# yifanlu0227/HEAL

Measured on AMD Instinct MI355X. Metric: scenes/sec (5-agent OPV2V-H, PointPillars+PyramidFusion), higher is better.
Workload: dtype f32

## Files before the change

### heal_amd/_capi.py

```python
import ctypes
import os
import re

HERE = os.path.dirname(os.path.abspath(__file__))
LIB_PATH = os.environ.get("HEAL_AMD_LIB") or os.path.join(HERE, "lib", "libheal_amd.so")
HEADER = os.path.join(os.path.dirname(HERE), "include", "heal_amd.h")
HEADER_EXPERIMENTAL = os.path.join(os.path.dirname(HERE), "include", "heal_amd_experimental.h")

_lib = None

c_void_p, c_int, c_float, c_size_t = ctypes.c_void_p, ctypes.c_int, ctypes.c_float, ctypes.c_size_t

_SIGNATURES = {
    "heal_abi_version": (c_int, []),
    "heal_last_error": (ctypes.c_char_p, []),
    "heal_fill_bytes": (c_int, [c_void_p, c_int, c_size_t, c_void_p]),
    "heal_next_launch_events": (c_int, [c_void_p, c_void_p]),
    "heal_voxelize_workspace": (c_size_t, [c_int, c_int, c_int, ctypes.c_longlong]),
    "heal_voxelize": (c_int, [c_void_p, c_int, c_void_p, c_void_p, c_int, c_int, c_int,
                              c_void_p, c_void_p, c_void_p, c_void_p, c_void_p, c_void_p, c_void_p, c_size_t, c_int, c_void_p]),
    "heal_voxelize_batch_workspace": (c_size_t, [c_int, c_int, c_int, c_int, ctypes.c_longlong]),
    "heal_voxelize_batch": (c_int, [c_void_p, c_void_p, c_int, c_void_p, c_void_p, c_int, c_int, c_void_p, c_void_p,
                                    c_void_p, c_void_p, c_void_p, c_size_t, c_int, c_void_p]),
    "heal_mask_points": (c_int, [c_void_p, c_int, c_void_p, c_int, c_void_p, c_void_p]),
# ... 44 lines not shown
                                  c_float, c_float, c_float, c_float, c_void_p, c_void_p]),
    "heal_pfn_moments": (c_int, [c_void_p, c_void_p, c_void_p, c_int, c_int, c_float, c_float, c_float, c_float, c_float, c_float,
                                 c_void_p, c_void_p]),
    "heal_pfn_backward": (c_int, [c_void_p, c_void_p, c_void_p, c_int, c_int, c_void_p, c_void_p, c_void_p, c_void_p, c_void_p,
                                  c_float, c_float, c_float, c_float, c_float, c_float, c_void_p, c_void_p, c_void_p]),
    "heal_mean_vfe": (c_int, [c_void_p, c_void_p, c_int, c_int, c_int, c_void_p, c_void_p, c_void_p]),
    "heal_sp_sort_workspace": (c_size_t, [c_int]),
    "heal_sp_sort_sites": (c_int, [c_void_p, c_int, c_void_p, c_int, c_void_p, c_void_p, c_void_p, c_size_t, c_void_p,
                                   c_void_p]),
    "heal_sp_wgrad_chunks": (c_int, [c_int]),
    "heal_sp_wgrad": (c_int, [c_void_p, c_void_p, c_void_p, c_int, c_int, c_int, c_int, c_void_p, c_void_p, c_void_p]),
    "heal_sp_gather_rows": (c_int, [c_void_p, c_void_p, c_int, c_int, c_void_p, c_void_p, c_void_p]),
    "heal_sp_table_capacity": (c_size_t, [c_int]),
    "heal_sp_hash_build": (c_int, [c_void_p, c_int, c_void_p, c_int, c_void_p, c_void_p, c_size_t, c_void_p, c_void_p]),
    "heal_sp_neighbors": (c_int, [c_void_p, c_int, c_void_p, c_void_p, c_void_p, c_void_p, c_void_p, c_int,
                                  c_void_p, c_void_p, c_size_t, c_void_p, c_void_p, c_void_p]),
    "heal_sp_out_sites_workspace": (c_size_t, [c_int, c_int]),
    "heal_sp_out_sites": (c_int, [c_void_p, c_int, c_void_p, c_void_p, c_void_p, c_void_p, c_void_p, c_int,
                                  c_void_p, c_int, c_void_p, c_void_p, c_size_t, c_void_p, c_void_p]),
    "heal_conv_gemm": (c_int, [c_void_p, c_void_p, c_void_p, c_void_p] + [c_int] * 8 + [c_void_p, c_void_p]),
    "heal_ln_stats": (c_int, [c_void_p, c_int, c_int, c_float, c_void_p, c_void_p]),
    "heal_linear": (c_int, [c_void_p, c_int, c_int, ctypes.c_longlong, c_void_p, c_void_p, c_void_p, c_int, c_void_p, c_int,
                            c_int, c_void_p, c_int, c_void_p, c_int, c_int, c_int, c_int, c_int, c_int, c_int,
                            ctypes.c_longlong, c_int, c_void_p]),
    "heal_split_attn_workspace": (c_size_t, [c_int, c_int, c_int]),
    "heal_split_attn_weights": (c_int, [c_void_p, ctypes.c_longlong, c_int, c_int, c_int] + [c_void_p] * 5 + [c_float] +
                                [c_void_p] * 5),
    "heal_split_attn_colsum": (c_int, [c_void_p, ctypes.c_longlong, c_int, c_int, c_int, c_void_p, c_void_p]),
    "heal_split_attn_weights_from_colsum": (c_int, [c_void_p, c_int, c_int, c_int, c_int] + [c_void_p] * 5 + [c_float] +
                                            [c_void_p] * 4),
    "heal_sp_rank_bytes": (c_size_t, [c_void_p, c_int]),
    "heal_sp_out_sites_rank": (c_int, [c_void_p, c_int, c_void_p, c_void_p, c_void_p, c_void_p, c_void_p, c_int,
                                       c_void_p, c_int, c_void_p, c_void_p, c_size_t, c_void_p, c_void_p, c_void_p]),
    "heal_sp_neighbors_rank": (c_int, [c_void_p, c_int, c_void_p, c_void_p, c_void_p, c_void_p, c_void_p, c_int,
                                       c_void_p, c_size_t, c_int, c_void_p, c_void_p, c_void_p, c_void_p]),
    "heal_sp_neighbors_root": (c_int, [c_void_p, c_int, c_void_p, c_void_p, c_void_p, c_void_p, c_void_p, c_int,
                                       c_void_p, c_size_t, c_int, c_void_p, c_void_p, c_void_p, c_void_p]),
    "heal_sp_root_rank_bytes": (c_size_t, [c_void_p, c_int]),
    "heal_sp_pair_tiles_words": (c_size_t, [c_int, c_int]),
    "heal_sp_neighbor_tiles": (c_int, [c_void_p, c_int, c_void_p, c_void_p, c_void_p, c_void_p, c_void_p, c_int,
                                       c_void_p, c_size_t, c_int, c_int, c_void_p, c_int, c_void_p, c_void_p, c_void_p]),
    "heal_sp_tiles_to_neighbors": (c_int, [c_void_p, c_int, c_int, c_void_p, c_void_p, c_void_p]),
    "heal_sp_conv_tiles_supported": (c_int, [c_int, c_int]),
    "heal_sp_conv_tiles": (c_int, [c_void_p, c_void_p, c_int, c_int, c_int, c_int, c_void_p, c_void_p, c_void_p, c_int,
                                   c_void_p, c_void_p, c_void_p]),
    "heal_sp_root_rank": (c_int, [c_void_p, c_int, c_void_p, c_int, c_void_p, c_void_p, c_void_p, c_int, c_void_p, c_void_p,
                                  c_size_t, c_void_p, c_void_p]),
    "heal_gconv_conv3_supported": (c_int, [c_int] * 5),
    "heal_gconv_conv3": (c_int, [c_void_p] * 6 + [c_int] * 7 + [c_void_p, c_void_p]),
    "heal_sp_transpose_neighbors": (c_int, [c_void_p, c_int, c_int, c_int, c_void_p, c_void_p, c_void_p]),
    "heal_sp_weight_fragments": (c_int, [c_void_p, c_int, c_int, c_int, c_void_p, c_void_p]),
    "heal_sp_conv": (c_int, [c_void_p, c_void_p, c_int, c_int, c_int, c_int, c_void_p, c_void_p, c_void_p, c_void_p, c_int,
                             c_void_p, c_void_p, c_void_p]),
    "heal_sp_to_bev_workspace": (c_size_t, [c_int, c_int, c_int, c_int]),
    "heal_sp_to_bev": (c_int, [c_void_p, c_void_p, c_int, c_int, c_void_p, c_int, c_void_p, c_void_p, c_size_t,
                               c_void_p, c_void_p]),
    "heal_agent_attention": (c_int, [c_void_p, c_void_p, c_void_p, c_void_p, c_int, c_int, c_int, c_int, c_float,
                                     c_int, c_void_p, c_int, c_void_p]),
    "heal_agent_attention_backward": (c_int, [c_void_p] * 5 + [c_int, c_int, c_int, c_int, c_float, c_int] + [c_void_p] * 3 +
                                      [c_int, c_void_p]),
    "heal_grouped_conv3x3": (c_int, [c_void_p, c_void_p, c_void_p, c_int, c_int, c_int, c_int, c_int, c_int, c_int,
                                     c_void_p, c_void_p]),
    "heal_bias_act": (c_int, [c_void_p, c_void_p, c_void_p, c_int, c_int, c_int, c_int, c_void_p]),
    "heal_resnext_bottleneck": (c_int, [c_void_p] * 7 + [c_int, c_int, c_int, c_int, c_void_p, c_void_p]),
    "heal_upsample2x_bilinear": (c_int, [c_void_p, c_int, c_int, c_int, c_int, c_void_p, c_void_p]),
    "heal_depthwise_conv": (c_int, [c_void_p, c_void_p, c_void_p] + [c_int] * 11 + [c_void_p, c_void_p, c_void_p]),
    "heal_camera_matrices": (c_int, [c_void_p] * 5 + [c_int, c_void_p, c_void_p]),
    "heal_channel_dot": (c_int, [c_void_p] * 3 + [c_int] * 3 + [c_void_p, c_void_p]),
    "heal_layernorm_nchw": (c_int, [c_void_p] * 3 + [c_int] * 3 + [c_float, c_void_p, c_void_p]),
    "heal_se_gate": (c_int, [c_void_p] * 5 + [c_int] * 3 + [c_float, c_int, c_void_p, c_void_p]),
    "heal_conv1x1": (c_int, [c_void_p] * 5 + [c_int] * 8 + [c_void_p, c_void_p]),
    "heal_stem7x7": (c_int, [c_void_p, ctypes.c_longlong, c_int, c_int, c_int, c_int, c_void_p, c_void_p, c_int, c_void_p, c_void_p]),
    "heal_conv1x1_split_supported": (c_int, [c_int] * 4),
    "heal_conv1x1_split": (c_int, [c_void_p] * 4 + [c_int] * 7 + [c_void_p, c_void_p]),
    "heal_conv1x1_tiled_supported": (c_int, [c_int] * 5),
    "heal_conv1x1_tiled": (c_int, [c_void_p] * 4 + [c_int] * 9 + [c_void_p, c_void_p]),
    "heal_conv1x1_splitk_workspace": (c_size_t, [c_int] * 5),
    "heal_conv1x1_splitk": (c_int, [c_void_p] * 5 + [c_int] * 7 + [c_void_p, c_void_p, c_size_t, c_void_p]),
    "heal_conv1x1_d2s": (c_int, [c_void_p] * 3 + [c_int] * 9 + [c_void_p, c_void_p]),
    "heal_conv3x3": (c_int, [c_void_p] * 4 + [c_int] * 7 + [c_void_p, c_void_p]),
    "heal_conv3x3_same": (c_int, [c_void_p] * 3 + [c_int] * 11 + [c_void_p, c_void_p]),
    "heal_grouped16_conv3x3": (c_int, [c_void_p] * 3 + [c_int] * 5 + [c_void_p, c_void_p]),
    "heal_grouped_small_conv3x3": (c_int, [c_void_p] * 3 + [c_int] * 7 + [c_void_p, c_void_p]),
    "heal_conv3x3_winograd4": (c_int, [c_void_p] * 4 + [c_int] * 6 + [c_void_p, c_void_p]),
    "heal_conv3x3_winograd": (c_int, [c_void_p] * 4 + [c_int] * 7 + [c_void_p, c_void_p]),
    "heal_conv3x3_winograd_kc": (c_int, [c_void_p] * 4 + [c_int] * 8 + [c_void_p, c_void_p]),
    "heal_conv3x3_winograd_splitk_workspace": (c_size_t, [c_int] * 5),
    "heal_conv3x3_winograd_splitk": (c_int, [c_void_p] * 4 + [c_int] * 8 + [c_void_p, c_void_p, c_size_t, c_void_p]),
    "heal_nms_quads_workspace": (c_size_t, [c_int]),
    "heal_nms_quads": (c_int, [c_void_p, c_int, c_float, c_void_p, c_size_t, c_void_p, c_void_p, c_void_p]),
    "heal_window_attention": (c_int, [c_void_p, c_void_p, c_int, c_int, c_int, c_int, c_int, c_int, c_float, c_void_p,
                                      c_void_p]),
    "heal_window_attention_backward_workspace": (c_size_t, [c_int, c_int, c_int, c_int]),
    "heal_window_attention_backward": (c_int, [c_void_p] * 4 + [c_int] * 6 + [c_float, c_void_p, c_void_p, c_void_p, c_size_t,
                                                c_void_p]),
    "heal_agent_window_attention": (c_int, [c_void_p, c_void_p] + [c_int] * 8 + [c_float, c_void_p, c_void_p]),
    "heal_agent_mean": (c_int, [c_void_p, c_int, ctypes.c_longlong, c_void_p, c_void_p]),
    "heal_v2v_message_workspace": (c_size_t, [c_int] * 5),
    "heal_v2v_message": (c_int, [c_void_p, c_void_p, c_void_p, ctypes.c_longlong, c_void_p, c_void_p] + [c_int] * 9
                         + [c_void_p, c_void_p, c_size_t, c_void_p]),
    "heal_gru_zero_state": (c_int, [c_void_p, ctypes.c_longlong, c_void_p, ctypes.c_longlong] + [c_int] * 4 + [c_void_p, c_void_p]),
    "heal_label_assign_workspace": (c_size_t, [c_int]),
    "heal_label_assign": (c_int, [c_void_p, c_int, c_void_p, c_int, c_float, c_float, c_void_p, c_void_p, c_void_p,
                                  c_size_t, c_void_p]),
    "heal_boxes_bev_matrix": (c_int, [c_void_p, c_int, c_void_p, c_int, c_int, c_void_p, c_void_p]),
    "heal_nms_bev_workspace": (c_size_t, [c_int]),
    "heal_nms_bev": (c_int, [c_void_p, c_int, c_float, c_int, c_void_p, c_size_t, c_void_p, c_void_p, c_void_p]),
    "heal_kd_kl_loss_workspace": (c_size_t, [c_int] * 4),
    "heal_kd_kl_loss": (c_int, [c_void_p, c_void_p] + [c_int] * 4 + [c_void_p, c_void_p, c_void_p, c_size_t, c_void_p]),
}


class HealAmdError(RuntimeError):
    pass


def declared_symbols(experimental=False):
    text = open(HEADER_EXPERIMENTAL if experimental else HEADER).read()
    text = re.sub(r"/\*.*?\*/", "", text, flags=re.S)
    return sorted(set(re.findall(r"\b(heal_[a-z0-9_]+)\s*\(", text)))


def abi_version_of_header():
    m = re.search(r"#define\s+HEAL_AMD_ABI_VERSION\s+(\d+)", open(HEADER).read())
    if not m:
        raise HealAmdError(f"{HEADER} does not define HEAL_AMD_ABI_VERSION")
    return int(m.group(1))


def lib():
    global _lib
    if _lib is None:
        if not os.path.exists(LIB_PATH):
            raise HealAmdError(
                f"{LIB_PATH} is missing: the HIP extension has not been built "
                "(run `python -m heal_amd.build`); heal_amd has no CPU fallback")
        import torch
        L = ctypes.CDLL(LIB_PATH)
        for name, (res, args) in _SIGNATURES.items():
            if not hasattr(L, name):
                continue
            f = getattr(L, name)
            f.restype = res
            f.argtypes = args
        want = abi_version_of_header()
        got = int(L.heal_abi_version()) if hasattr(L, "heal_abi_version") else -1
        if got != want:
            raise HealAmdError(f"{LIB_PATH} has C-ABI version {got}, include/heal_amd.h declares {want}: rebuild it "
                               "(python -m heal_amd.build --force)")
        _lib = L
    return _lib


_TRACE = int(os.environ.get("HEAL_TRACE_CALLS", "0") or 0)


def _trace_call(name, args):
    import sys
    import torch
    cap = torch.cuda.is_current_stream_capturing()
    extra = ""
    if _TRACE >= 2:
        extra = " " + " ".join(hex(a.value or 0) if isinstance(a, ctypes.c_void_p) else str(a) for a in args
                               if isinstance(a, (int, float, ctypes.c_void_p)))
    print(f"[heal pid {os.getpid()}] {'capture ' if cap else ''}{name}{extra}", file=sys.stderr, flush=True)

# ... 103 lines not shown
```

### heal_amd/opencood/models/sub_modules/bev_blocks.py

```python
import numpy as np
import torch
import torch.nn as nn
import torch.nn.functional as F

from heal_amd.derived import derived


def fold_bn(conv, bn, transposed=False):
    def build():
        scale = bn.weight / torch.sqrt(bn.running_var + bn.eps)
        shift = bn.bias - bn.running_mean * scale
        if transposed:
            w = conv.weight * scale.view(1, -1, 1, 1)
        else:
            w = conv.weight * scale.view(-1, 1, 1, 1)
        b = shift if conv.bias is None else shift + conv.bias * scale
        return w.contiguous(), b.contiguous()
    return derived("fold_bn", (conv.weight, conv.bias, bn.weight, bn.bias, bn.running_mean, bn.running_var), build, (transposed,))


import os
_CONV1X1 = os.environ.get("HEAL_CONV1X1", "1") == "1"
_CONV3X3 = os.environ.get("HEAL_CONV3X3", "1") == "1"

# ... 59 lines not shown
    if module.training and torch.is_grad_enabled():
        raise NotImplementedError(
            f"{type(module).__name__}: no gradient path (the sparse-convolution encoder is inference-only in this build). "
            "Call model.eval() and run under torch.no_grad(), or freeze this module (eval mode, input without gradient).")


class ConvBN(nn.Module):

    @staticmethod
    def run(x, conv, bn, relu, residual=None, out=None):
        if out is not None and not grad_path(x, bn, conv):
            w, b = fold_bn(conv, bn)
            y = conv_bias_act(x, w, b, conv.stride, conv.padding, conv.dilation, conv.groups, relu, residual, out=out)
            if y.data_ptr() != out.data_ptr():
                out.copy_(y)
            return out
        if out is not None:
            return out.copy_(ConvBN.run(x, conv, bn, relu, residual))
        if grad_path(x, bn, conv):
            y = bn(conv(x))
            if residual is not None:
                y = y + residual
            return F.relu(y) if relu else y
        w, b = fold_bn(conv, bn)
        return conv_bias_act(x, w, b, conv.stride, conv.padding, conv.dilation, conv.groups, relu, residual)


def conv3x3(in_planes, out_planes, stride=1, groups=1, dilation=1):
    return nn.Conv2d(in_planes, out_planes, kernel_size=3, stride=stride, padding=dilation, groups=groups,
                     bias=False, dilation=dilation)


def conv1x1(in_planes, out_planes, stride=1):
    return nn.Conv2d(in_planes, out_planes, kernel_size=1, stride=stride, bias=False)


class BasicBlock(nn.Module):
    expansion = 1

    def __init__(self, inplanes, planes, stride=1, downsample=None, groups=1, base_width=64, dilation=1,
                 norm_layer=None):
        super().__init__()
        norm_layer = norm_layer or nn.BatchNorm2d
        if groups != 1 or base_width != 64:
            raise ValueError("BasicBlock only supports groups=1 and base_width=64")
        self.conv1 = conv3x3(inplanes, planes, stride)
        self.bn1 = norm_layer(planes)
        self.relu = nn.ReLU(inplace=True)
        self.conv2 = conv3x3(planes, planes)
        self.bn2 = norm_layer(planes)
        self.downsample = downsample
        self.stride = stride

    def takes_pooled(self):
        d = self.downsample
        return (d is not None and isinstance(d[0], nn.Conv2d) and d[0].kernel_size == (1, 1) and d[0].stride == (2, 2)
                and d[0].padding == (0, 0) and d[0].out_channels == 64 and d[0].bias is None
                and self.conv1.stride == (2, 2) and self.conv1.out_channels == 64 and self.conv1.in_channels % 32 == 0
                and isinstance(self.bn1, nn.BatchNorm2d) and isinstance(d[1], nn.BatchNorm2d))

    def _stem_params(self, x):
        from heal_amd import ops
        w1, b1 = fold_bn(self.conv1, self.bn1)
        wd, bd = fold_bn(self.downsample[0], self.downsample[1])
        frag = getattr(x, "fragments", ops.stem_fragments)
        return derived("stem_block", (w1, b1, wd, bd), lambda: frag(w1, wd) + (b1, bd), (getattr(x, "weight_layout", "tiles"),))

    def forward(self, x):
        from heal_amd import ops
        if isinstance(x, (ops.PooledBEV, ops.PillarBEV)):
            if (not grad_path(None, self) and self.takes_pooled() and x.channels == self.conv1.in_channels
                    and x.stem_supported(self.conv1.out_channels, self.downsample[0].out_channels)):
                wm, wd, b1, bd = self._stem_params(x)
                out, identity = x.stem_block(wm, b1, wd, bd)
                return ConvBN.run(out, self.conv2, self.bn2, relu=True, residual=identity)
            x = x.dense()
        identity = x
        if self.downsample is not None:
            identity = ConvBN.run(x, self.downsample[0], self.downsample[1], relu=False)
        out = ConvBN.run(x, self.conv1, self.bn1, relu=True)
        return ConvBN.run(out, self.conv2, self.bn2, relu=True, residual=identity)


class Bottleneck(nn.Module):
    expansion = 4

    def __init__(self, inplanes, planes, stride=1, downsample=None, groups=1, base_width=64, dilation=1,
                 norm_layer=None, expansion=None):
        super().__init__()
        norm_layer = norm_layer or nn.BatchNorm2d
        exp = self.expansion if expansion is None else expansion
        width = int(planes * (base_width / 64.0)) * groups
        self.conv1 = conv1x1(inplanes, width)
        self.bn1 = norm_layer(width)
        self.conv2 = conv3x3(width, width, stride, groups, dilation)
        self.bn2 = norm_layer(width)
        self.conv3 = conv1x1(width, planes * exp)
        self.bn3 = norm_layer(planes * exp)
        self.relu = nn.ReLU(inplace=True)
        self.downsample = downsample
        self.stride = stride

    def _fused_params(self):
        from heal_amd import ops
        w1, b1 = fold_bn(self.conv1, self.bn1)
        w2, b2 = fold_bn(self.conv2, self.bn2)
        w3, b3 = fold_bn(self.conv3, self.bn3)
        return derived("resnext_bottleneck", (w1, b1, w2, b2, w3, b3), lambda: (
            ops.mfma_a_fragments(w1.reshape(w1.shape[0], w1.shape[1])), b1, w2, b2,
            ops.mfma_a_fragments(w3.reshape(w3.shape[0], w3.shape[1])), b3))

    def _fusable(self, x):
        import os
        if os.environ.get("HEAL_FUSED_BOTTLENECK", "0") != "1":
            return False
        from heal_amd import ops
        if not ops.experimental_build():
            return False
        c = self.conv1.in_channels
        return (x.is_cuda and self.downsample is None and self.stride == 1 and self.conv2.groups == 32
                and self.conv3.out_channels == c and self.conv1.out_channels == 2 * c and c in (64, 128, 256)
                and self.conv2.dilation == (1, 1))

    def out_shape(self, x):
        s = self.stride
        return (int(x.shape[0]), self.conv3.out_channels, (int(x.shape[2]) - 1) // s + 1, (int(x.shape[3]) - 1) // s + 1)

    def forward(self, x, out=None):
        if not grad_path(x, self) and self._fusable(x):
            from heal_amd import ops
            y = ops.resnext_bottleneck(x.contiguous(), *self._fused_params())
            return y if out is None else out.copy_(y)
        identity = x
        if self.downsample is not None:
            identity = ConvBN.run(x, self.downsample[0], self.downsample[1], relu=False)
        y = ConvBN.run(x, self.conv1, self.bn1, relu=True)
        y = ConvBN.run(y, self.conv2, self.bn2, relu=True)
        return ConvBN.run(y, self.conv3, self.bn3, relu=True, residual=identity, out=out)


class ResNetModified(nn.Module):

    def __init__(self, block, layers, layer_strides, num_filters, groups=1, width_per_group=64, inplanes=64,
                 expansion=None):
        super().__init__()
        self.inplanes = inplanes
        self.groups = groups
        self.base_width = width_per_group
        self.layernum = len(num_filters)
        self._exp = block.expansion if expansion is None else expansion
        for i in range(self.layernum):
            setattr(self, f"layer{i}", self._make_layer(block, num_filters[i], layers[i], layer_strides[i]))
        for m in self.modules():
            if isinstance(m, nn.Conv2d):
                nn.init.kaiming_normal_(m.weight, mode="fan_out", nonlinearity="relu")

    def _make_layer(self, block, planes, blocks, stride):
        exp = self._exp
        kw = {"expansion": exp} if block is Bottleneck else {}
        downsample = None
        if stride != 1 or self.inplanes != planes * exp:
            downsample = nn.Sequential(conv1x1(self.inplanes, planes * exp, stride), nn.BatchNorm2d(planes * exp))
        layers = [block(self.inplanes, planes, stride, downsample, self.groups, self.base_width, 1, None, **kw)]
        self.inplanes = planes * exp
        for _ in range(1, blocks):
            layers.append(block(self.inplanes, planes, groups=self.groups, base_width=self.base_width, **kw))
        return nn.Sequential(*layers)

    @staticmethod
    def stage_chunk(layer, x):
        mb = float(os.environ.get("HEAL_STAGE_CHUNK_MB", "0"))
        if mb <= 0 or not x.is_cuda or torch.is_grad_enabled() or not all(isinstance(b, Bottleneck) for b in layer):
            return 0
        n = int(x.shape[0])
        blk = layer[-1]
        co, s0 = blk.conv3.out_channels, layer[0].stride
        ho, wo = (int(x.shape[2]) - 1) // s0 + 1, (int(x.shape[3]) - 1) // s0 + 1
        per_agent = 4.0 * ho * wo * (2 * co + 2 * blk.conv1.out_channels) / 2 ** 20
        chunk = max(1, int(mb // per_agent))
        return chunk if chunk < n else 0

    def run_stage(self, layer, x):
        chunk = self.stage_chunk(layer, x)
        if not chunk:
            return layer(x)
        n = int(x.shape[0])
        shape = list(x.shape)
        for blk in layer:
            shape = list(blk.out_shape(torch.empty(shape, device="meta")))
        y = torch.empty(shape, dtype=x.dtype, device=x.device)
        for a in range(0, n, chunk):
            xa = x[a:a + chunk]
            for j, blk in enumerate(layer):
                xa = blk(xa, out=y[a:a + chunk]) if j == len(layer) - 1 else blk(xa)
        return y

    def forward(self, x):
        feats = []
        for i in range(self.layernum):
            x = self.run_stage(getattr(self, f"layer{i}"), x)
            feats.append(x)
        return feats


class _Deblock(nn.Sequential):

    def __init__(self, conv, bn):
        super().__init__(conv, bn, nn.ReLU())

    def out_shape(self, x):
        conv = self[0]
        if isinstance(conv, nn.ConvTranspose2d):
            return conv.out_channels, int(x.shape[2]) * conv.stride[0], int(x.shape[3]) * conv.stride[1]
        s0, s1 = conv.stride
        return conv.out_channels, (int(x.shape[2]) - conv.kernel_size[0]) // s0 + 1, (int(x.shape[3]) - conv.kernel_size[1]) // s1 + 1

    def forward(self, x, into=None):
        y = self._forward(x, into)
        if into is not None and y.data_ptr() != into[0][:, into[1]:].data_ptr():
            dst = into[0][:, into[1]:into[1] + y.shape[1]]
# ... 253 lines not shown
```

### heal_amd/ops.py

```python
import ctypes
import os

import numpy as np
import torch

from . import _capi, derived
from .derived import derived as _derived

_WS = {}

TIMING = None
SP_TRACE = None
LAST_CALLS = None


def _remember(name, fn):
    if LAST_CALLS is not None:
        LAST_CALLS[name] = fn


def graph_period_ms(fn, reps=20, iters=10):
    global TIMING, LAST_CALLS
    saved = (TIMING, LAST_CALLS)
    TIMING, LAST_CALLS = None, None
# ... 1687 lines not shown


def split_attn_weights(branches, groups, rows_per_group, w_out, b_out, fc1, ln_g, ln_b, eps, fc2):
    branches = _need(branches, torch.float32, "branches")
    C = int(branches.shape[-1])
    dev = branches.device
    ws = _workspace("split_attn", _capi.query("heal_split_attn_workspace", groups, rows_per_group, C), dev)
    scale = torch.empty((groups, 3, C), dtype=torch.float32, device=dev)
    bias = torch.empty((groups, C), dtype=torch.float32, device=dev)
    _capi.call("heal_split_attn_weights", _ptr(branches), int(branches.stride(0)), groups, rows_per_group, C, _ptr(w_out),
               _ptr(b_out), _ptr(fc1), _ptr(ln_g), _ptr(ln_b), float(eps), _ptr(fc2), _ptr(ws), _ptr(scale), _ptr(bias),
               _stream())
    return scale, bias


def split_attn_colsum(branches, groups, rows_per_group):
    branches = _need(branches, torch.float32, "branches")
    C = int(branches.shape[-1])
    out = torch.empty((groups, 3, (rows_per_group + 511) // 512, C), dtype=torch.float32, device=branches.device)
    _capi.call("heal_split_attn_colsum", _ptr(branches), int(branches.stride(0)), groups, rows_per_group, C, _ptr(out), _stream())
    return out


def split_attn_weights_from_colsum(colsum, rows_per_part, w_out, b_out, fc1, ln_g, ln_b, eps, fc2):
    colsum = _need(colsum, torch.float32, "colsum")
    n_parts, groups, _three, chunks, C = (int(v) for v in colsum.shape)
    if chunks != (rows_per_part + 511) // 512:
        raise ValueError(f"split_attn_weights_from_colsum: {chunks} chunks do not match {rows_per_part} rows per part")
    dev = colsum.device
    scale = torch.empty((groups, 3, C), dtype=torch.float32, device=dev)
    bias = torch.empty((groups, C), dtype=torch.float32, device=dev)
    _capi.call("heal_split_attn_weights_from_colsum", _ptr(colsum), n_parts, groups, int(rows_per_part), C, _ptr(w_out),
               _ptr(b_out), _ptr(fc1), _ptr(ln_g), _ptr(ln_b), float(eps), _ptr(fc2), _ptr(scale), _ptr(bias), _stream())
    return scale, bias


def grouped16_fragments(weight, cg):
    def build():
        C = int(weight.shape[0])
        w = weight.detach().reshape(C // 16, 16, cg, 9)
        if cg == 16:
            full = w
        else:
            full = torch.zeros((C // 16, 16, 16, 9), dtype=w.dtype, device=w.device)
            full[:, :8, :8] = w[:, :8]
            full[:, 8:, 8:] = w[:, 8:]
        return full.reshape(C // 16, 16, 4, 4, 9).permute(0, 4, 2, 3, 1).contiguous()
    return _derived("grouped16_fragments", (weight,), build)


def grouped_small_fragments(weight, cg):
    C = int(weight.shape[0])
    return _derived("grouped_small_fragments", (weight,),
                    lambda: weight.detach().reshape(C // 16, 16, cg, 9).permute(0, 3, 2, 1).contiguous())


def grouped_conv3x3(x, weight, bias, groups, stride=1, relu=True):
    import os
    x = _need(x, torch.float32, "x")
    weight = _need(weight, torch.float32, "weight")
    n, C, H, W = (int(v) for v in x.shape)
    bias = _need_bias(bias, C, "grouped_conv3x3")
    Ho, Wo = (H + 2 - 3) // stride + 1, (W + 2 - 3) // stride + 1
    y = torch.empty((n, C, Ho, Wo), dtype=torch.float32, device=x.device)
    cg = C // groups
    mode = os.environ.get("HEAL_GCONV_MFMA", "1")
    if C % 16 == 0 and W % 4 == 0 and Wo % 4 == 0 and mode in ("1", "s") and cg in (4, 8, 16):
        frag = grouped_small_fragments(weight, cg)
        with _Timed(f"grouped_conv3x3_c{C}" + ("_s2" if stride == 2 else ""), 2.0 * 9 * n * C * cg * Ho * Wo,
                    4.0 * n * C * (H * W + Ho * Wo), kernel_events=True):
            _capi.call("heal_grouped_small_conv3x3", _ptr(x), _ptr(frag), _ptr(bias), n, C, cg, H, W, int(stride),
                       int(bool(relu)), _ptr(y), _stream())
        return y
    if stride == 1 and C % 16 == 0 and W % 4 == 0 and ((cg == 16 and mode != "0") or (cg == 8 and mode == "8")):
        frag = grouped16_fragments(weight, cg)
        with _Timed(f"grouped_conv3x3_c{C}", 2.0 * 9 * n * C * cg * Ho * Wo, 4.0 * n * C * (H * W + Ho * Wo)):
            _capi.call("heal_grouped16_conv3x3", _ptr(x), _ptr(frag), _ptr(bias), n, C, H, W, int(bool(relu)), _ptr(y),
                       _stream())
        return y
    with _Timed(f"grouped_conv3x3_c{C}" + ("_s2" if stride == 2 else ""), 2.0 * 9 * n * C * (C // groups) * Ho * Wo,
                4.0 * n * C * (H * W + Ho * Wo)):
        _capi.call("heal_grouped_conv3x3", _ptr(x), _ptr(weight), _ptr(bias), n, C, int(groups), H, W, int(stride),
                   int(bool(relu)), _ptr(y), _stream())
    return y


def gconv_conv3_supported(width, cg, cout, H, W):
    return bool(_capi.query("heal_gconv_conv3_supported", int(width), int(cg), int(cout), int(H), int(W)))


def gconv_conv3(x, w2, b2, groups, w3, b3, residual=None, relu=True):
    x = _need(x, torch.float32, "x")
    n, width, H, W = (int(v) for v in x.shape)
    cg = width // groups
    cout = int(w3.shape[0])
    frag2 = grouped_small_fragments(_need(w2, torch.float32, "w2"), cg)
    frag3 = _derived("gconv_conv3_fragments", (w3,), lambda: mfma_a_fragments(w3.detach().reshape(cout, width)))
    y = torch.empty((n, cout, H, W), dtype=torch.float32, device=x.device)
    flops = 2.0 * n * H * W * (9 * width * cg + width * cout)
    nbytes = 4.0 * n * H * W * (width + cout * (2 if residual is not None else 1))
    with _Timed(f"gconv_conv3_{width}_{cout}", flops, nbytes, kernel_events=True):
        _capi.call("heal_gconv_conv3", _ptr(x), _ptr(frag2), _ptr(_need(b2, torch.float32, "b2")), _ptr(frag3),
                   _ptr(_need(b3, torch.float32, "b3")), _optr(residual), n, width, cg, cout, H, W, int(bool(relu)), _ptr(y), _stream())
    return y


def bias_act_(x, bias=None, residual=None, relu=True):
    x = _need(x, torch.float32, "x")
    n, C = int(x.shape[0]), int(x.shape[1])
    HW = int(x.shape[2] * x.shape[3])
    if residual is not None:
        residual = _need(residual, torch.float32, "residual")
    _capi.call("heal_bias_act", _ptr(x), _ptr(bias), _ptr(residual), n, C, HW, int(bool(relu)), _stream())
    return x


def mfma_a_fragments(wm):
    M, K = wm.shape
    return wm.reshape(M // 16, 16, K // 4, 4).permute(0, 2, 3, 1).reshape(M // 16, K // 4, 64).contiguous()


def conv1x1_fragments(w):
    def build():
        cout, cin = int(w.shape[0]), int(w.shape[1])
        mpad, kpad = (cout + 63) // 64 * 64, (cin + 31) // 32 * 32
        wm = w.detach().reshape(cout, cin)
        if (mpad, kpad) != (cout, cin):
            wm = torch.nn.functional.pad(wm, (0, kpad - cin, 0, mpad - cout))
        fr = mfma_a_fragments(wm)
        return fr.reshape(mpad // 16, kpad // 16, 4, 64).permute(0, 1, 3, 2).contiguous()
    return _derived("conv1x1_fragments", (w,), build)


def conv1x1_supported(cin, cout, hw, stride=1, out_w=None):
    if stride == 1:
        return hw % 4 == 0 and hw >= 64
    return stride == 2 and out_w is not None and out_w % 4 == 0 and hw >= 64


def conv1x1_ksplit(n, cin, cout, hw):
    chunks = (cin + 31) // 32
    blocks = -(-cout // 64) * -(-hw // 64) * n
    env = os.environ.get("HEAL_C1_KSPLIT")
    want = int(env) if env is not None else (min(chunks // 2, max(2, 256 // blocks)) if blocks < 128 and chunks >= 8 else 1)
    if want < 2 or chunks < 2 or hw % 4:
        return 1
    want = min(want, chunks, 65535 // n)
    return -(-chunks // -(-chunks // want))


def stem7x7_fragments(w):
    cout, cin = int(w.shape[0]), int(w.shape[1])
    if cout != 64 or tuple(w.shape[2:]) != (7, 7) or not 1 <= cin <= 4:
        raise _capi.HealAmdError(f"stem7x7: weight must be [64, 1..4, 7, 7], got {tuple(w.shape)}")

    def build():
        K = cin * 49
        ks = (K + 3) // 4
        wk = torch.nn.functional.pad(w.detach().to(torch.float32).reshape(64, K), (0, 4 * ks - K))
        return wk.reshape(4, 16, ks, 4).permute(0, 2, 3, 1).contiguous()
    return _derived("stem7x7_fragments", (w,), build)


def stem7x7(x, w, bias, pool=True):
    x = _need(x, torch.float32, "x")
    n, cx, H, W = (int(v) for v in x.shape)
# ... 425 lines not shown
```

### include/heal_amd.h

```cpp
#ifndef HEAL_AMD_H
#define HEAL_AMD_H

#include <stddef.h>
#include <stdint.h>

#ifdef __cplusplus
extern "C" {
#endif

#define HEAL_AMD_ABI_VERSION 12

int heal_abi_version(void);
const char* heal_last_error(void);

int heal_fill_bytes(void* dst, int byte, size_t bytes, void* stream);
int heal_next_launch_events(void* start_event, void* stop_event);

size_t heal_voxelize_workspace(int n_points, int max_points, int max_voxels, long long agents_x_cells);
int heal_voxelize(const float* points, int n_points,
                  const float* range_host, const float* voxel_size_host,
                  int max_points, int max_voxels, int batch_idx,
                  float* voxels, int32_t* coords, int32_t* num_points, int32_t* n_voxels,
                  const int32_t* row_offset, int32_t* row_offset_next,
                  void* ws, size_t ws_bytes, int tables_clean, void* stream);
// ... 162 lines not shown
int heal_sp_conv_tiles(const float* feat_in, const uint32_t* tiles, int n_out, int slot_sites, int c_in, int c_out,
                       const float* weight_frag, const float* bn_scale, const float* bn_shift, int relu, float* feat_out,
                       const int32_t* n_out_dev, void* stream);
int heal_sp_transpose_neighbors(const int32_t* nbr, int n_out, int kernel_volume, int n_in, int32_t* nbr_t,
                                const int32_t* n_out_dev, void* stream);
int heal_sp_wgrad_chunks(int n_out);
int heal_sp_wgrad(const float* feat_in, const float* grad_out, const int32_t* nbr, int n_out, int kernel_volume, int c_in,
                  int c_out, const int32_t* n_out_dev, float* partials, void* stream);
int heal_sp_weight_fragments(const float* weight, int kernel_volume, int c_in, int c_out, float* out, void* stream);
int heal_sp_conv(const float* feat_in, const int32_t* nbr, int n_out, int kernel_volume, int c_in, int c_out,
                 const float* weight, const float* weight_frag, const float* bn_scale, const float* bn_shift,
                 int relu, float* feat_out, const int32_t* n_out_dev, void* stream);
size_t heal_sp_to_bev_workspace(int batch, int D, int H, int W);
int heal_sp_to_bev(const float* features, const int32_t* indices, int n, int channels,
                   const int32_t* shape_host, int batch, float* out, void* ws, size_t ws_bytes,
                   const int32_t* n_dev, void* stream);

int heal_bev_pool_backward(const float* grad_cells, const float* depth_logit, const float* feat, const float* frustum,
                           const float* cam_mats, int n_agents, int n_cams, int D, int fH, int fW, int channels,
                           const float* dx_host, const float* bx_host, const int32_t* nx_host, float* grad_logit,
                           float* grad_feat, void* stream);

int heal_agent_attention(const float* q, const float* k, const float* v, const int32_t* key_mask, int n_pix,
                         int n_agents, int channels, int heads, float scale, int out_rows, float* out,
                         int agent_major ,
                         void* stream);
int heal_agent_attention_backward(const float* q, const float* k, const float* v, const int32_t* key_mask,
                                  const float* grad_out, int n_pix, int n_agents, int channels, int heads, float scale,
                                  int out_rows, float* grad_q, float* grad_k, float* grad_v, int agent_major, void* stream);

int heal_grouped_conv3x3(const float* x, const float* weight, const float* bias, int n, int channels, int groups,
                         int H, int W, int stride, int relu, float* y, void* stream);
int heal_bias_act(float* x, const float* bias, const float* residual, int n, int channels, int HW, int relu,
                  void* stream);

int heal_upsample2x_bilinear(const float* x, int n, int channels, int H, int W, float* y, void* stream);

int heal_depthwise_conv(const float* x, const float* weight, const float* bias, int n, int channels, int H, int W,
                        int ksize, int stride, int pad_t, int pad_l, int Ho, int Wo, int act, float* y,
                        float* channel_sums, void* stream);

int heal_layernorm_nchw(const float* x, const float* gamma, const float* beta, int n, int channels, int HW, float eps,
                        float* y, void* stream);

int heal_channel_dot(const float* x, const float* weight, const float* bias, int n, int channels, int HW, float* y,
                     void* stream);

int heal_se_gate(const float* mean, const float* w_reduce, const float* b_reduce, const float* w_expand_t,
                 const float* b_expand, int n, int channels, int squeezed, float scale, int tiles, float* gate,
                 void* stream);

int heal_conv1x1(const float* x, const float* weight_frag, const float* bias, const float* residual,
                 const float* in_scale, int n, int cin, int cout, int H, int W, int stride, int act,
                 int out_pixel_major, float* y, void* stream);

int heal_conv3x3_same(const float* x, const float* weight_frag, const float* bias, int n, int cin, int cout, int H, int W,
                      int stride, int pad_t, int pad_l, int Ho, int Wo, int act, float* y, void* stream);

int heal_stem7x7(const float* x, long long image_stride, int n, int cin, int H, int W, const float* weight_frag,
                 const float* bias, int pool, float* y, void* stream);
int heal_conv1x1_split_supported(int cin, int cout, int H, int W);
int heal_conv1x1_split(const float* x, const void* weight_frag, const float* bias, const float* residual, int n, int cin, int cout,
                       int H, int W, int act, int n_products, float* y, void* stream);
size_t heal_conv1x1_splitk_workspace(int n, int cout, int H, int W, int ksplit);
int heal_conv1x1_splitk(const float* x, const float* weight_frag, const float* bias, const float* residual,
                        const float* in_scale, int n, int cin, int cout, int H, int W, int act, int ksplit, float* y, void* ws,
                        size_t ws_bytes, void* stream);

int heal_conv1x1_d2s(const float* x, const float* weight_frag, const float* bias, int n, int cin, int cout, int H, int W,
                     int act, int k, int dst_channels, int dst_channel_offset, float* y, void* stream);

int heal_conv3x3(const float* x, const float* weight_frag, const float* bias, const float* residual, int n, int cin,
                 int cout, int H, int W, int stride, int relu, float* y, void* stream);

int heal_conv_gemm(const float* x, const float* weight_tap_major, const float* bias, const float* residual, int n, int cin,
                   int cout, int H, int W, int ksize, int stride, int relu, float* y, void* stream);

int heal_grouped16_conv3x3(const float* x, const float* weight_frag, const float* bias, int n, int channels, int H, int W,
                           int relu, float* y, void* stream);

int heal_grouped_small_conv3x3(const float* x, const float* weight_q, const float* bias, int n, int channels,
                               int group_channels, int H, int W, int stride, int relu, float* y, void* stream);

int heal_conv3x3_winograd(const float* x, const float* u_frag, const float* bias, const float* residual, int n, int cin,
                          int cout, int H, int W, int relu, int waves, float* y, void* stream);
int heal_conv3x3_winograd_kc(const float* x, const float* u_frag, const float* bias, const float* residual, int n, int cin,
                             int cout, int H, int W, int relu, int waves, int kc, float* y, void* stream);
size_t heal_conv3x3_winograd_splitk_workspace(int n, int cout, int H, int W, int ksplit);
int heal_conv3x3_winograd_splitk(const float* x, const float* u_frag, const float* bias, const float* residual, int n, int cin,
                                 int cout, int H, int W, int relu, int waves, int ksplit, float* y, void* ws, size_t ws_bytes,
                                 void* stream);

int heal_boxes_bev_matrix(const float* boxes_a, int n, const float* boxes_b, int m, int mode, float* out,
                          void* stream);
size_t heal_nms_bev_workspace(int n);
int heal_nms_bev(const float* boxes_sorted, int n, float thresh, int rotated, void* workspace,
                 size_t workspace_bytes, long long* keep, int* num_keep, void* stream);

size_t heal_nms_quads_workspace(int n);
int heal_nms_quads(const float* quads_sorted, int n, float thresh, void* workspace, size_t workspace_bytes,
                   long long* keep, int* num_keep, void* stream);

int heal_window_attention(const float* qkv, const float* pos_bias, int n_agents, int H, int W, int heads,
                          int dim_head, int window, float scale, float* out, void* stream);
size_t heal_window_attention_backward_workspace(int n_agents, int H, int W, int heads);
int heal_window_attention_backward(const float* qkv, const float* pos_bias, const float* out, const float* grad_out, int n_agents,
                                   int H, int W, int heads, int dim_head, int window, float scale, float* grad_qkv,
                                   float* grad_bias, void* ws, size_t ws_bytes, void* stream);

int heal_agent_window_attention(const float* qkv, const float* bias, int n_agents, int n_valid, int H, int W, int heads,
                                int dim_head, int window, int mode, float scale, float* out, void* stream);
int heal_agent_mean(const float* x, int n_agents, long long n_elems, float* out, void* stream);

size_t heal_v2v_message_workspace(int n_ego, int cout, int H, int W, int nsplit);
int heal_v2v_message(const float* xs, const float* mask, const float* e, long long e_stride, const float* w_frag,
                     const float* residual, int n_ego, int n_agents, int cin, int cout, int H, int W, int mode, int nsplit,
                     int tile_h, float* out, void* ws, size_t ws_bytes, void* stream);
int heal_gru_zero_state(const float* gates, long long gates_stride, const float* add, long long add_stride, int n, int channels,
                        int H, int W, float* h, void* stream);

int heal_ln_stats(const float* x, int n_tokens, int channels, float eps, float* stats, void* stream);
int heal_linear(const float* x, int lda, int x_part_cols, long long x_part_stride, const float* ln_stats,
                const float* weight, const float* bias,
                int bias_per_group, const float* colscale, int colscale_part, int group_rows, const float* residual,
                int ldr, float* out, int ldo, int n_tokens, int n_out, int n_in, int map_inner, int map_outer,
                int part_cols, long long part_stride, int act, void* stream);
size_t heal_split_attn_workspace(int groups, int rows_per_group, int channels);
int heal_split_attn_weights(const float* branches, long long part_stride, int groups, int rows_per_group, int channels,
                            const float* w_out, const float* b_out, const float* fc1, const float* ln_gamma,
                            const float* ln_beta, float eps, const float* fc2, float* colsum_ws, float* scale,
                            float* bias, void* stream);
int heal_split_attn_colsum(const float* branches, long long part_stride, int groups, int rows_per_group, int channels,
                           float* colsum, void* stream);
int heal_split_attn_weights_from_colsum(const float* colsum, int n_parts, int groups, int rows_per_part, int channels,
                                        const float* w_out, const float* b_out, const float* fc1, const float* ln_gamma,
                                        const float* ln_beta, float eps, const float* fc2, float* scale, float* bias,
                                        void* stream);

size_t heal_label_assign_workspace(int n_gt);
int heal_label_assign(const float* anchor_boxes, int n_anchors, const float* gt_boxes, int n_gt,
                      float pos_threshold, float neg_threshold, int32_t* assigned, uint8_t* neg, void* ws,
                      size_t ws_bytes, void* stream);

size_t heal_kd_kl_loss_workspace(int n, int channels, int H, int W);
int heal_kd_kl_loss(const float* student, const float* teacher, int n, int channels, int H, int W, float* loss, float* grad,
                    void* ws, size_t ws_bytes, void* stream);

#ifdef __cplusplus
}
#endif
#endif
```

Measured before the change: 161.2.

## Fuse bottleneck 1x1 conv with grouped 3x3 conv in one HIP kernel

Adds a kernel that computes the bottleneck's conv1 (1x1, BN-folded, ReLU) for a haloed tile into LDS with MFMA, then immediately runs the 32-group 3x3 conv2 from LDS, for specific ResNeXt block shapes. This removes the global-memory write and re-read of the intermediate activation and one kernel launch. In exchange the halo pixels of conv1 are recomputed across neighbouring tiles. The path is gated on a fixed set of shapes and environment flags.

```diff
diff --git a/heal_amd/_capi.py b/heal_amd/_capi.py
--- a/heal_amd/_capi.py
+++ b/heal_amd/_capi.py
@@ -150,6 +150,7 @@
     "heal_conv3x3_same": (c_int, [c_void_p] * 3 + [c_int] * 11 + [c_void_p, c_void_p]),
     "heal_grouped16_conv3x3": (c_int, [c_void_p] * 3 + [c_int] * 5 + [c_void_p, c_void_p]),
     "heal_grouped_small_conv3x3": (c_int, [c_void_p] * 3 + [c_int] * 7 + [c_void_p, c_void_p]),
+    "heal_conv1_gconv3x3": (c_int, [c_void_p] * 5 + [c_int] * 7 + [c_void_p, c_void_p]),
     "heal_conv3x3_winograd4": (c_int, [c_void_p] * 4 + [c_int] * 6 + [c_void_p, c_void_p]),
     "heal_conv3x3_winograd": (c_int, [c_void_p] * 4 + [c_int] * 7 + [c_void_p, c_void_p]),
     "heal_conv3x3_winograd_kc": (c_int, [c_void_p] * 4 + [c_int] * 8 + [c_void_p, c_void_p]),
diff --git a/heal_amd/csrc/conv1_gconv.hip b/heal_amd/csrc/conv1_gconv.hip
--- /dev/null
+++ b/heal_amd/csrc/conv1_gconv.hip
@@ -0,0 +1,235 @@
+#include <stdlib.h>
+#include "common.h"
+#include "../../include/heal_amd.h"
+
+namespace heal {
+
+using f32x4 = __attribute__((ext_vector_type(4))) float;
+
+template <int CG, int TH, int STRIDE, int PF>
+__global__ __launch_bounds__(256) __attribute__((amdgpu_waves_per_eu(PF == 1 && TH == 8 && STRIDE == 1 ? 4 : 3, PF == 1 && TH == 8 && STRIDE == 1 ? 5 : 4))) void k_conv1_gconv(
+    const float* __restrict__ x, const float* __restrict__ w1frag, const float* __restrict__ b1, const float* __restrict__ wq,
+    const float* __restrict__ b2, int Cin, int width, int H, int W, int Ho, int Wo, int tiles_x, float* __restrict__ y) {
+    static_assert(CG == 4 || CG == 8 || CG == 16, "4, 8 or 16 channels per group");
+    static_assert(TH == 8 || TH == 16, "tile height");
+    static_assert(STRIDE == 1 || STRIDE == 2, "stride");
+    static_assert(PF == 1 || PF == 2, "chunks in flight per block");
+    constexpr int TW = STRIDE == 1 ? 32 : 16, NSEG = TW / 16, RW = TH / 4;
+    constexpr int PR = STRIDE * TH + 3 - STRIDE, PC = STRIDE * TW + 3 - STRIDE;
+    constexpr int NSIDE = 3 - STRIDE;
+    constexpr int NSTEP = 9 * CG;
+    constexpr int KH = CG == 16 ? 2 : 1;
+    constexpr int CGH = CG / KH;
+    constexpr int NB = CG / 4, NBH = CGH / 4;
+    static_assert(STRIDE * TW == 32, "a patch row is 32 interior pixels + halo");
+    constexpr int KC = 8;
+    constexpr int RS = 36;
+    constexpr int LD = (PR * RS - 16 + 31) / 32 * 32 + 16;
+    constexpr int NPIX = PR * PC, NT = (NPIX + 15) / 16, NTW = (NT + 3) / 4;
+    constexpr int SP4 = NPIX * 4, SX4 = 2 * KC * LD / 4, SA4 = SP4 > SX4 ? SP4 : SX4, SW4 = NSTEP * 16 / 4;
+    static_assert((SA4 + SW4) * 16 <= 80 * 1024, "two blocks per CU");
+    __shared__ float4 smem[SA4 + SW4];
+    float4* const sP = smem;
+    float* const sX = reinterpret_cast<float*>(smem);
+    float4* const sW = smem + SA4;
+
+    const Block3 bk = xcd_block();
+    const int sg = bk.x, n = bk.z;
+    const int ty = bk.y / tiles_x, tx = bk.y - ty * tiles_x;
+    const int oy0 = ty * TH, ox0 = tx * TW;
+    const int gy0 = oy0 * STRIDE - 1, gx0 = ox0 * STRIDE;
+    const int t = threadIdx.x, wave = t >> 6, l = t & 63;
+    const int lk = l >> 4, ln = l & 15;
+    const size_t HW = (size_t)H * W, HWo = (size_t)Ho * Wo;
+    const float* __restrict__ xin = x + (size_t)n * Cin * HW;
+
+    constexpr int IT_W = (SW4 + 255) / 256;
+#pragma unroll
+    for (int it = 0; it < IT_W; ++it) {
+        const int i = min(t + 256 * it, SW4 - 1);
+        sW[i] = reinterpret_cast<const float4*>(wq + (size_t)sg * NSTEP * 16)[i];
+    }
+
+    constexpr int N_IN = PR * KC * 8, IT_IN = (N_IN + 255) / 256;
+    constexpr int N_HA = PR * KC * NSIDE, IT_HA = (N_HA + 255) / 256;
+    int g_in[IT_IN], s_in[IT_IN], g_ha[IT_HA], s_ha[IT_HA];
+#pragma unroll
+    for (int it = 0; it < IT_IN; ++it) {
+        const int u = min(t + 256 * it, N_IN - 1);
+        const int quad = u & 7, ch = (u >> 3) & 7, row = u >> 6;
+        const int gy = gy0 + row, gx = gx0 + quad * 4;
+        const bool ok = gy >= 0 && gy < H && gx < W;
+        g_in[it] = ch * (int)HW + (ok ? gy * W + gx : 0);
+        s_in[it] = ch * LD + row * RS + quad * 4;
+    }
+#pragma unroll
+    for (int it = 0; it < IT_HA; ++it) {
+        const int u = min(t + 256 * it, N_HA - 1);
+        const int ch = u & 7, side = NSIDE == 2 ? (u >> 3) & 1 : 0, row = u / (8 * NSIDE);
+        const int gy = gy0 + row, gx = side ? gx0 + 32 : gx0 - 1;
+        const bool ok = gy >= 0 && gy < H && gx >= 0 && gx < W;
+        g_ha[it] = ch * (int)HW + (ok ? gy * W + gx : 0);
+        s_ha[it] = ch * LD + row * RS + 32 + side;
+    }
+    f32x4 st_in[PF][IT_IN];
+    float st_ha[PF][IT_HA];
+    auto load_chunk = [&](int c, f32x4 (&vi)[IT_IN], float (&vh)[IT_HA]) {
+        const float* __restrict__ src = xin + (size_t)c * KC * HW;
+#pragma unroll
+        for (int it = 0; it < IT_IN; ++it) vi[it] = *reinterpret_cast<const f32x4*>(src + g_in[it]);
+#pragma unroll
+        for (int it = 0; it < IT_HA; ++it) vh[it] = src[g_ha[it]];
+    };
+    auto store_chunk = [&](int buf, const f32x4 (&vi)[IT_IN], const float (&vh)[IT_HA]) {
+        float* dst = sX + buf * KC * LD;
+#pragma unroll
+        for (int it = 0; it < IT_IN; ++it) *reinterpret_cast<f32x4*>(dst + s_in[it]) = vi[it];
+#pragma unroll
+        for (int it = 0; it < IT_HA; ++it) dst[s_ha[it]] = vh[it];
+    };
+    int b_off[NTW];
+#pragma unroll
+    for (int i = 0; i < NTW; ++i) {
+        const int j = min((wave + 4 * i) * 16 + ln, NPIX - 1);
+        const int row = j / PC, col = j - row * PC;
+        b_off[i] = lk * LD + row * RS + (col == 0 ? 32 : (NSIDE == 2 && col == PC - 1) ? 33 : col - 1);
+    }
+    f32x4 t1[NTW];
+#pragma unroll
+    for (int i = 0; i < NTW; ++i) t1[i] = f32x4{0.f, 0.f, 0.f, 0.f};
+
+    const int nch = Cin / KC, nq = Cin / 16;
+    const float4* __restrict__ afrag = reinterpret_cast<const float4*>(w1frag) + (size_t)sg * nq * 64 + l;
+    float4 a_cur = afrag[0], a_nxt = a_cur;
+    load_chunk(0, st_in[0], st_ha[0]);
+    if (PF == 2) load_chunk(1, st_in[PF - 1], st_ha[PF - 1]);
+    store_chunk(0, st_in[0], st_ha[0]);
+    lds_barrier();
+    for (int q = 0; q < nq; ++q) {
+#pragma unroll
+        for (int h = 0; h < 2; ++h) {
+            const int c = 2 * q + h;
+            if (h == 0 && q + 1 < nq) a_nxt = afrag[(size_t)(q + 1) * 64];
+            if (c + PF < nch) load_chunk(c + PF, st_in[h & (PF - 1)], st_ha[h & (PF - 1)]);
+            const float* __restrict__ bsrc = sX + h * KC * LD;
+#pragma unroll
+            for (int ks = 0; ks < 2; ++ks) {
+                const float a = h == 0 ? (ks == 0 ? a_cur.x : a_cur.y) : (ks == 0 ? a_cur.z : a_cur.w);
+                float bv[NTW];
+#pragma unroll
+                for (int i = 0; i < NTW; ++i) bv[i] = bsrc[ks * 4 * LD + b_off[i]];
+#pragma unroll
+                for (int i = 0; i < NTW; ++i)
+                    if (wave + 4 * i < NT) t1[i] = __builtin_amdgcn_mfma_f32_16x16x4f32(a, bv[i], t1[i], 0, 0, 0);
+            }
+            if (c + 1 < nch) store_chunk(h ^ 1, st_in[(h ^ 1) & (PF - 1)], st_ha[(h ^ 1) & (PF - 1)]);
+            lds_barrier();
+        }
+        a_cur = a_nxt;
+    }
+    {
+        const float4 bq = *reinterpret_cast<const float4*>(b1 + sg * 16 + lk * 4);
+#pragma unroll
+        for (int i = 0; i < NTW; ++i) {
+            const int j = (wave + 4 * i) * 16 + ln;
+            if (j >= NPIX) continue;
+            const int row = j / PC, col = j - row * PC;
+            const int gy = gy0 + row, gx = gx0 - 1 + col;
+            const bool in = gy >= 0 && gy < H && gx >= 0 && gx < W;
+            sP[j * 4 + lk] = make_float4(in ? fmaxf(t1[i][0] + bq.x, 0.f) : 0.f, in ? fmaxf(t1[i][1] + bq.y, 0.f) : 0.f,
+                                         in ? fmaxf(t1[i][2] + bq.z, 0.f) : 0.f, in ? fmaxf(t1[i][3] + bq.w, 0.f) : 0.f);
+        }
+    }
+    __syncthreads();
+
+    const float bv0 = b2[sg * 16 + (l & 15)];
+    const int p = (l >> 4) * 4 + (l & 3);
+    const int unit0 = (((l >> 2) & 3) * 4 / CG) * NB;
+    const float4* __restrict__ abase = sP + ((wave * RW * STRIDE) * PC + p * STRIDE) * 4 + unit0;
+    f32x4 acc[RW][NSEG];
+#pragma unroll
+    for (int o = 0; o < RW; ++o)
+#pragma unroll
+        for (int s = 0; s < NSEG; ++s) acc[o][s] = f32x4{0.f, 0.f, 0.f, 0.f};
+#pragma unroll
+    for (int half = 0; half < KH; ++half) {
+        float wreg[9 * CGH];
+#pragma unroll
+        for (int tap = 0; tap < 9; ++tap)
+#pragma unroll
+            for (int ci = 0; ci < CGH; ++ci)
+                wreg[tap * CGH + ci] = reinterpret_cast<const float*>(sW)[(tap * CG + half * CGH + ci) * 16 + (l & 15)];
+#pragma unroll
+        for (int ry = 0; ry < STRIDE * (RW - 1) + 3; ++ry) {
+#pragma unroll
+            for (int dx = 0; dx < 3; ++dx) {
+                float4 av[NSEG][NBH];
+#pragma unroll
+                for (int s = 0; s < NSEG; ++s)
+#pragma unroll
+                    for (int hh = 0; hh < NBH; ++hh) av[s][hh] = abase[(ry * PC + s * 16 * STRIDE + dx) * 4 + half * NBH + hh];
+#pragma unroll
+                for (int ci = 0; ci < CGH; ++ci) {
+#pragma unroll
+                    for (int o = 0; o < RW; ++o) {
+                        const int dy = ry - STRIDE * o;
+                        if (dy < 0 || dy > 2) continue;
+#pragma unroll
+                        for (int s = 0; s < NSEG; ++s) {
+                            const float4 qv = av[s][ci >> 2];
+                            const float a = (ci & 3) == 0 ? qv.x : (ci & 3) == 1 ? qv.y : (ci & 3) == 2 ? qv.z : qv.w;
+                            acc[o][s] = __builtin_amdgcn_mfma_f32_4x4x1f32(a, wreg[(dy * 3 + dx) * CGH + ci], acc[o][s], 0, 0, 0);
+                        }
+                    }
+                }
+            }
+        }
+    }
+    float* __restrict__ yout = y + ((size_t)n * width + (size_t)sg * 16 + (l & 15)) * HWo;
+#pragma unroll
+    for (int o = 0; o < RW; ++o) {
+        const int oy = oy0 + wave * RW + o;
+#pragma unroll
+        for (int s = 0; s < NSEG; ++s) {
+            const int ox = ox0 + s * 16 + (l >> 4) * 4;
+            if (oy >= Ho || ox >= Wo) continue;
+            float4 v = make_float4(acc[o][s][0] + bv0, acc[o][s][1] + bv0, acc[o][s][2] + bv0, acc[o][s][3] + bv0);
+            v.x = fmaxf(v.x, 0.f); v.y = fmaxf(v.y, 0.f); v.z = fmaxf(v.z, 0.f); v.w = fmaxf(v.w, 0.f);
+            *reinterpret_cast<float4*>(yout + (size_t)oy * Wo + ox) = v;
+        }
+    }
+}
+
+}
+
+using namespace heal;
+
+extern "C" int heal_conv1_gconv3x3(const float* x, const float* w1_frag, const float* b1, const float* weight_q, const float* b2,
+                                   int n, int cin, int width, int group_channels, int H, int W, int stride, float* y, void* stream) {
+    HEAL_REQUIRE(group_channels == 4 || group_channels == 8 || group_channels == 16,
+                 "conv1_gconv3x3: 4, 8 or 16 channels per group (got %d)", group_channels);
+    HEAL_REQUIRE(width == 32 * group_channels, "conv1_gconv3x3: 32 groups (width %d != 32 * %d)", width, group_channels);
+    HEAL_REQUIRE(stride == 1 || stride == 2, "conv1_gconv3x3: stride must be 1 or 2 (got %d)", stride);
+    HEAL_REQUIRE(n >= 1 && n <= 65535 && H >= 1 && W >= 4 && cin >= 32 && cin % 32 == 0,
+                 "conv1_gconv3x3: needs Cin %% 32 == 0 and 1 <= n <= 65535 (got Cin=%d n=%d H=%d W=%d)", cin, n, H, W);
+    const int Ho = (H - 1) / stride + 1, Wo = (W - 1) / stride + 1;
+    HEAL_REQUIRE(W % 4 == 0 && Wo % 4 == 0, "conv1_gconv3x3: W and the output width must be multiples of 4 (got W=%d Wo=%d)", W, Wo);
+    HEAL_REQUIRE((long long)H * W * 8 < (1ll << 31), "conv1_gconv3x3: map too large (%d x %d)", H, W);
+    HEAL_REQUIRE(x && w1_frag && b1 && weight_q && b2 && y, "conv1_gconv3x3: null pointer");
+    HEAL_REQUIRE((((uintptr_t)x | (uintptr_t)w1_frag | (uintptr_t)b1 | (uintptr_t)weight_q | (uintptr_t)b2 | (uintptr_t)y) & 15) == 0,
+                 "conv1_gconv3x3: every pointer must be 16-B aligned");
+    const int th = (group_channels == 4 && stride == 1) ? 16 : 8;
+    const int tw = stride == 1 ? 32 : 16;
+    const int tiles_x = ceil_div(Wo, tw), tiles_y = ceil_div(Ho, th);
+    HEAL_REQUIRE((long long)tiles_x * tiles_y <= 65535, "conv1_gconv3x3: grid limit");
+    const dim3 grid(width / 16, tiles_x * tiles_y, n);
+    hipStream_t s_ = (hipStream_t)stream;
+#define HEAL_CG(CG_, TH_, ST_, PF_)                                                                                   \
+    if (group_channels == CG_ && th == TH_ && stride == ST_)                                                          \
+        HEAL_LAUNCH_EV((k_conv1_gconv<CG_, TH_, ST_, PF_>), grid, dim3(256), 0, s_, x, w1_frag, b1, weight_q, b2, cin, width, H, W, Ho, Wo, \
+                       tiles_x, y);
+    HEAL_CG(4, 16, 1, 2) HEAL_CG(8, 8, 1, 1) HEAL_CG(16, 8, 1, 1) HEAL_CG(4, 8, 2, 2) HEAL_CG(8, 8, 2, 2) HEAL_CG(16, 8, 2, 2)
+#undef HEAL_CG
+    HEAL_LAUNCH_CHECK();
+    return 0;
+}
diff --git a/heal_amd/opencood/models/sub_modules/bev_blocks.py b/heal_amd/opencood/models/sub_modules/bev_blocks.py
--- a/heal_amd/opencood/models/sub_modules/bev_blocks.py
+++ b/heal_amd/opencood/models/sub_modules/bev_blocks.py
@@ -165,6 +165,13 @@
         return ConvBN.run(out, self.conv2, self.bn2, relu=True, residual=identity)
 
 
+CONV1_GCONV_SITES = frozenset({
+    (2, 64, 128, 1, 144, 144),
+    (3, 64, 256, 2, 256, 256),
+    (2, 64, 256, 2, 192, 192),
+})
+
+
 class Bottleneck(nn.Module):
     expansion = 4
 
@@ -205,6 +212,24 @@
                 and self.conv3.out_channels == c and self.conv1.out_channels == 2 * c and c in (64, 128, 256)
                 and self.conv2.dilation == (1, 1))
 
+    def _front_fused(self, x):
+        from heal_amd import ops
+        mode = os.environ.get("HEAL_CONV1_GCONV", "1")
+        c1, c2 = self.conv1, self.conv2
+        if (mode == "0" or not _CONV1X1 or not x.is_cuda or x.dtype != torch.float32 or x.dim() != 4 or c2.groups != 32
+                or c1.out_channels != c2.in_channels or c1.kernel_size != (1, 1) or c1.stride != (1, 1) or c1.padding != (0, 0)
+                or c2.kernel_size != (3, 3) or c2.padding != (1, 1) or c2.dilation != (1, 1) or c2.stride not in ((1, 1), (2, 2))
+                or not isinstance(self.bn1, nn.BatchNorm2d) or not isinstance(self.bn2, nn.BatchNorm2d)):
+            return False
+        n, cin, H, W = (int(v) for v in x.shape)
+        width, s = c1.out_channels, c2.stride[0]
+        if c1.in_channels != cin or not ops.conv1_gconv3x3_supported(cin, width, 32, H, W, s) or x.data_ptr() % 16:
+            return False
+        if (os.environ.get("HEAL_GCONV_MFMA", "1") not in ("1", "s") or ops.arith_products() or ops.conv1x1_tiled_ok(n, cin, width, H * W)
+                or ops.conv1x1_ksplit(n, cin, width, H * W) != 1 or not ops.conv1x1_supported(cin, width, H * W)):
+            return False
+        return mode == "force" or (n, cin, width, s, H, W) in CONV1_GCONV_SITES
+
     def out_shape(self, x):
         s = self.stride
         return (int(x.shape[0]), self.conv3.out_channels, (int(x.shape[2]) - 1) // s + 1, (int(x.shape[3]) - 1) // s + 1)
@@ -217,8 +242,14 @@
         identity = x
         if self.downsample is not None:
             identity = ConvBN.run(x, self.downsample[0], self.downsample[1], relu=False)
-        y = ConvBN.run(x, self.conv1, self.bn1, relu=True)
-        y = ConvBN.run(y, self.conv2, self.bn2, relu=True)
+        if not grad_path(x, self) and self._front_fused(x):
+            from heal_amd import ops
+            w1, b1 = fold_bn(self.conv1, self.bn1)
+            w2, b2 = fold_bn(self.conv2, self.bn2)
+            y = ops.conv1_gconv3x3(x, w1, b1, w2, b2, 32, self.conv2.stride[0])
+        else:
+            y = ConvBN.run(x, self.conv1, self.bn1, relu=True)
+            y = ConvBN.run(y, self.conv2, self.bn2, relu=True)
         return ConvBN.run(y, self.conv3, self.bn3, relu=True, residual=identity, out=out)
 
 
diff --git a/heal_amd/ops.py b/heal_amd/ops.py
--- a/heal_amd/ops.py
+++ b/heal_amd/ops.py
@@ -1793,6 +1793,39 @@
                 4.0 * n * C * (H * W + Ho * Wo)):
         _capi.call("heal_grouped_conv3x3", _ptr(x), _ptr(weight), _ptr(bias), n, C, int(groups), H, W, int(stride),
                    int(bool(relu)), _ptr(y), _stream())
+    return y
+
+
+def conv1_gconv3x3_supported(cin, width, groups, H, W, stride=1):
+    if groups != 32 or stride not in (1, 2) or width % groups:
+        return False
+    Wo = (W - 1) // stride + 1
+    return width // groups in (4, 8, 16) and cin >= 32 and cin % 32 == 0 and W % 4 == 0 and Wo % 4 == 0
+
+
+def conv1_gconv3x3(x, w1, b1, w2, b2, groups=32, stride=1):
+    x = _need(x, torch.float32, "x")
+    w1 = _need(w1, torch.float32, "w1")
+    w2 = _need(w2, torch.float32, "w2")
+    n, cin, H, W = (int(v) for v in x.shape)
+    width = int(w1.shape[0])
+    if int(w1.shape[1]) != cin or int(w2.shape[0]) != width or width % groups or int(w2.shape[1]) != width // groups:
+        raise _capi.HealAmdError(f"conv1_gconv3x3: weight shapes {tuple(w1.shape)} / {tuple(w2.shape)} do not fit x {tuple(x.shape)}")
+    if groups != 32:
+        raise _capi.HealAmdError(f"conv1_gconv3x3: 32 groups only (got {groups})")
+    cg = width // groups
+    b1 = _need_bias(b1, width, "conv1_gconv3x3")
+    b2 = _need_bias(b2, width, "conv1_gconv3x3")
+    if b1 is None or b2 is None:
+        raise _capi.HealAmdError("conv1_gconv3x3: both biases are required")
+    frag1 = conv1x1_fragments(w1)
+    frag2 = grouped_small_fragments(w2, cg)
+    Ho, Wo = (H - 1) // stride + 1, (W - 1) // stride + 1
+    y = torch.empty((n, width, Ho, Wo), dtype=torch.float32, device=x.device)
+    with _Timed(f"conv1_gconv_{cin}_{width}" + ("_s2" if stride == 2 else ""),
+                2.0 * n * width * (cin * H * W + 9 * cg * Ho * Wo), 4.0 * n * (cin * H * W + width * Ho * Wo), kernel_events=True):
+        _capi.call("heal_conv1_gconv3x3", _ptr(x), _ptr(frag1), _ptr(b1), _ptr(frag2), _ptr(b2), n, cin, width, cg, H, W,
+                   int(stride), _ptr(y), _stream())
     return y
 
 
diff --git a/include/heal_amd.h b/include/heal_amd.h
--- a/include/heal_amd.h
+++ b/include/heal_amd.h
@@ -268,6 +268,9 @@
 int heal_grouped_small_conv3x3(const float* x, const float* weight_q, const float* bias, int n, int channels,
                                int group_channels, int H, int W, int stride, int relu, float* y, void* stream);
 
+int heal_conv1_gconv3x3(const float* x, const float* w1_frag, const float* b1, const float* weight_q, const float* b2, int n,
+                        int cin, int width, int group_channels, int H, int W, int stride, float* y, void* stream);
+
 int heal_conv3x3_winograd(const float* x, const float* u_frag, const float* bias, const float* residual, int n, int cin,
                           int cout, int H, int W, int relu, int waves, float* y, void* stream);
 int heal_conv3x3_winograd_kc(const float* x, const float* u_frag, const float* bias, const float* residual, int n, int cin,
```

After: 162.2 (median of 4 runs). About the same (+0.6%).
